# EthanD11/RS-VIO

Measured on AMD Instinct MI355X. Metric: stereo frames/sec (tracker+BA) on 752×480 EuRoC stream; BA ms/iter at window=10, higher is better.
Workload: dtype f32 (tracker) / f64 (BA)

## Files before the change

### rs-vio_amd/csrc/ba.hip

```cpp
#include <rccl/rccl.h>

#include <algorithm>
#include <chrono>
#include <cmath>
#include <cstdlib>
#include <cstring>
#include <string>
#include <sys/resource.h>
#include <numeric>
#include <stdexcept>
#include <vector>

#include "common.hpp"

#include "ba_envelope.hpp"
#include "obs_pass.hpp"
#include "se3.hpp"
#include "wave.hpp"

#pragma clang fp contract(fast)

namespace rsvio {

namespace {
// ... 1742 lines not shown
        __builtin_amdgcn_fence(__ATOMIC_ACQUIRE, "");
    }
    __syncthreads();
    const double* mine = p2p_slot(P.peer[me], par, 0);
    double sums[kE];
#pragma unroll
    for (int i = 0; i < kE; ++i) sums[i] = 0.0;
    if (nr <= 2)
        p2p_group_sums_own<kE, 2>(mine, nr, me, ne, tid, T, own, sums);
    else if (nr <= 4)
        p2p_group_sums_own<kE, 4>(mine, nr, me, ne, tid, T, own, sums);
    else
        p2p_group_sums_own<kE, 8>(mine, nr, me, ne, tid, T, own, sums);
#pragma unroll
    for (int i = 0; i < kE; ++i) {
        const int e = tid + T * i;
        if (e >= ne) break;
        const double a = sums[i];
        const int d = dst[i];
        if (d >= 0)
            M[d & (kMfMapLambda - 1)] = a;
        else if (d <= -2)
            gsh[-2 - d] = a;
    }
    if (tid == 0) {
        double cv[kP2PMax], fv[kP2PMax];
#pragma unroll
        for (int r = 0; r < kP2PMax; ++r) {
            const bool peer = r < nr && r != me;
            cv[r] = peer ? __hip_atomic_load(mine + (size_t)r * kP2PMsg + ne, __ATOMIC_RELAXED, __HIP_MEMORY_SCOPE_SYSTEM)
                         : osc[0];
            fv[r] = peer ? __hip_atomic_load(mine + (size_t)r * kP2PMsg + ne + 1, __ATOMIC_RELAXED,
                                             __HIP_MEMORY_SCOPE_SYSTEM)
                         : osc[1];
        }
        double c = 0.0, f = 0.0;
#pragma unroll
        for (int r = 0; r < kP2PMax; ++r)
            if (r < nr) {
                c += cv[r];
                f += fv[r];
            }
        Wk.sys[ne] = c;
        *fail = f != 0.0;
        *xgen = gen;
    }
    if (tid < nr && P.xnw)
        P.xnw[tid] = tid == me ? G.n_wave
                               : (int)__hip_atomic_load(mine + (size_t)tid * kP2PMsg + ne + 2, __ATOMIC_RELAXED,
                                                        __HIP_MEMORY_SCOPE_SYSTEM);
    return false;
}

template <int H, int J, int PW, bool KD = false>
__device__ __forceinline__ void mf_pivot(double (&a)[kMfPanel], double (&uq)[kMfPanel], double lp, double inv,
                                         double* Lf, double* Up, int lane, bool& bad, double* Dv = nullptr) {
    constexpr int K = kMfPanel * H + J;
    const double u = a[J];
    if constexpr (KD)
        if (lane == 0) Dv[K] = inv;
    double inv_next = 1.0;
    double uk1 = 0.0;
    if constexpr (J + 1 < PW) {
        uk1 = rl64(u, K + 1);
        const double piv = fma(-(uk1 * uk1), inv, rl64(a[J + 1], K + 1));
        bad |= !(piv > 0.0) || !isfinite(piv);
#ifndef RSVIO_K5_RCP_LATE
        double y0 = __builtin_amdgcn_rcp(piv);
        __asm__ volatile("" : "+v"(y0));
        const double e = fma(-piv, y0, 1.0);
        inv_next = fma(y0, fma(e, e, e), y0);
#else
        inv_next = rcp_f64(piv);
#endif
    }
    const double l = u * inv;
    if constexpr (J + 1 < PW) a[J + 1] = fma(-l, uk1, a[J + 1]);
    __builtin_amdgcn_sched_barrier(0);
    if constexpr (J > 0)
#pragma unroll
        for (int jj = J + 2; jj < PW; ++jj) a[jj] = fma(-lp, uq[jj], a[jj]);
    if constexpr (J + 2 < PW) a[J + 2] = fma(-l, rl64(u, K + 2), a[J + 2]);
    Lf[K * kMfLd + lane] = l;
    Up[J * kMfLd + lane] = u;
#ifndef RSVIO_K5_LDSQ
#pragma unroll
    for (int jj = J + 3; jj < PW; ++jj) uq[jj] = rl64(u, kMfPanel * H + jj);
#else
#pragma unroll
    for (int jj = J + 3; jj < PW; ++jj) uq[jj] = Up[J * kMfLd + kMfPanel * H + jj];
#endif
    if constexpr (J + 1 < PW) mf_pivot<H, J + 1, PW, KD>(a, uq, l, inv_next, Lf, Up, lane, bad, Dv);
}

template <int NF, int H, bool KD = false>
__device__ __forceinline__ void mf_factor(const double* M, double* Lf, double* Uh, int lane, bool& bad,
                                          double* Dv = nullptr) {
    constexpr int NP = MfDims<NF>::NP;
    constexpr int C0 = kMfPanel * H;
    constexpr int PW = (NP - C0) < kMfPanel ? (NP - C0) : kMfPanel;
    double a[kMfPanel], uq[kMfPanel];
#pragma unroll
    for (int jj = 0; jj < kMfPanel; ++jj) {
        a[jj] = jj < PW ? M[(C0 + jj) * kMfLd + lane] : 0.0;
        uq[jj] = 0.0;
    }
    const double piv = rl64(a[0], C0);
    bad |= !(piv > 0.0) || !isfinite(piv);
    mf_pivot<H, 0, PW, KD>(a, uq, 0.0, rcp_f64(piv), Lf, Uh, lane, bad, Dv);
}

template <int NF, int H>
__device__ __forceinline__ void mf_update(double* M, const double* Lf, const double* Uh, int lane, int wid, int nw,
                                          int J0, int J1) {
    constexpr int NT = MfDims<NF>::NT;
    constexpr int C0 = kMfPanel * H;
    const int i16 = lane & 15, k4 = lane >> 4;
    int ntile = 0;
    for (int J = J0; J < J1; ++J) ntile += NT - J;
    for (int t = wid; t < ntile; t += nw) {
        int TJ = J0, rem = t;
        while (rem >= NT - TJ) {
            rem -= NT - TJ;
            ++TJ;
        }
        const int TI = TJ + rem;
        double av[2], bv[2];
#pragma unroll
        for (int m = 0; m < 2; ++m) {
            const int kk = 4 * m + k4;
            av[m] = -Uh[kk * kMfLd + 16 * TI + i16];
            bv[m] = Lf[(C0 + kk) * kMfLd + 16 * TJ + i16];
        }
        mf_dbl4 c;
#pragma unroll
        for (int r = 0; r < 4; ++r) c[r] = M[(16 * TJ + i16) * kMfLd + 16 * TI + k4 + 4 * r];
        c = __builtin_amdgcn_mfma_f64_16x16x4f64(av[0], bv[0], c, 0, 0, 0);
        c = __builtin_amdgcn_mfma_f64_16x16x4f64(av[1], bv[1], c, 0, 0, 0);
#pragma unroll
        for (int r = 0; r < 4; ++r) M[(16 * TJ + i16) * kMfLd + 16 * TI + k4 + 4 * r] = c[r];
    }
}

template <int NF, int H, bool KD = false>
__device__ __forceinline__ void mf_panel(double* M, double* Lf, double* Up, int tid, bool& bad, double* Dv = nullptr) {
    constexpr int NT = MfDims<NF>::NT, NH = MfDims<NF>::NH;
    constexpr int C0 = kMfPanel * H;
    const int lane = tid & 63, wave = tid >> 6;
    if constexpr (H == 0) STAMP(9); else if constexpr (H == 2) STAMP(15); else if constexpr (H == 4) STAMP(30);
    if constexpr (H + 1 == NH) STAMP(7);
    if constexpr (H + 1 < NH) {
        constexpr int T0 = (C0 + kMfPanel) / 16;
        double* Uh = Up + (H & 1) * kMfPanel * kMfLd;
        if (wave == 0) {
            mf_update<NF, H>(M, Lf, Uh, lane, 0, 1, T0, T0 + 1);
            __builtin_amdgcn_fence(__ATOMIC_SEQ_CST, "wavefront");
            __builtin_amdgcn_wave_barrier();
            mf_factor<NF, H + 1, KD>(M, Lf, Up + ((H + 1) & 1) * kMfPanel * kMfLd, lane, bad, Dv);
        } else {
            mf_update<NF, H>(M, Lf, Uh, lane, wave - 1, kK5Threads / 64 - 1, T0 + 1, NT);
        }
        __syncthreads();
        if constexpr (H == 0) STAMP(13); else if constexpr (H == 2) STAMP(19); else if constexpr (H == 4) STAMP(31);
        mf_panel<NF, H + 1, KD>(M, Lf, Up, tid, bad, Dv);
    }
}

#ifdef RSVIO_STAMPS
#define WSTAMP(w, k)                                                                           \
    do {                                                                                       \
        if (threadIdx.x == 64 * (w) && blockIdx.x < 4096) {                                    \
            __builtin_amdgcn_s_waitcnt(0);                                                     \
            g_dbg[blockIdx.x * 32 + (k)] = (unsigned long long)clock64();                      \
        }                                                                                      \
    } while (0)
#else
#define WSTAMP(w, k) \
    do {             \
    } while (0)
#endif

template <int NF>
struct BkDims {
    static constexpr int NP = 6 * NF;
    static constexpr int RPL = NP + 1 <= 64 ? 1 : 2;
    static constexpr int NT = (NP + 1 + 15) / 16;
    static constexpr int NPP = 16 * NT;
    static constexpr int NTC = (NP + 15) / 16;
    static constexpr int LD = NF <= 10 ? kMfLd : kBkLd;
};

template <int NF, int K, int NWU>
__device__ __forceinline__ void bk_update(double* M, const double* Uk, int lane, int wid, int env) {
    using D = BkDims<NF>;
    constexpr int c0 = 6 * K, cmin = c0 + 12;
    if constexpr (cmin < D::NP) {
        constexpr int TJ0 = cmin / 16;
        constexpr int ntile_dense = (D::NTC - TJ0) * D::NT - (D::NTC - 1 + TJ0) * (D::NTC - TJ0) / 2;
        constexpr int Q = (ntile_dense + NWU - 1) / NWU;
        constexpr int TIb = D::NP / 16;
        const int rlast = min(6 * (env + 1), D::NP) - 1;
        const int TIe = rlast / 16;
        const int TJe = env >= K + 2 ? min(TIe, D::NTC - 1) : TJ0 - 1;
        const int extra = TIb > TIe ? 1 : 0;
        int ntile = 0;
        for (int TJ = TJ0; TJ <= TJe; ++TJ) ntile += TIe - TJ + 1 + extra;
        const int i16 = lane & 15, k4 = lane >> 4;
        double av[Q][2], bv[Q][2];
        mf_dbl4 c[Q];
        int base[Q];
        bool live[Q];
#pragma unroll
        for (int q = 0; q < Q; ++q) {
            const int t = wid + NWU * q;
            int TJ = TJ0, rem = t < ntile ? t : 0;
            while (rem >= TIe - TJ + 1 + extra) {
                rem -= TIe - TJ + 1 + extra;
                ++TJ;
            }
            const int TI = rem <= TIe - TJ ? TJ + rem : TIb;
            const int col = 16 * TJ + i16;
            live[q] = t < ntile && col >= cmin && col < D::NP;
            base[q] = col * D::LD + 16 * TI + k4;
#pragma unroll
            for (int m = 0; m < 2; ++m) {
                const int kk = 4 * m + k4;
                av[q][m] = kk < 6 ? -Uk[kk * D::LD + 16 * TI + i16] : 0.0;
                bv[q][m] = (kk < 6 && live[q]) ? M[(c0 + kk) * D::LD + col] : 0.0;
            }
#pragma unroll
            for (int r = 0; r < 4; ++r) c[q][r] = live[q] ? M[base[q] + 4 * r] : 0.0;
        }
#pragma unroll
        for (int q = 0; q < Q; ++q)
            if (wid + NWU * q < ntile) c[q] = __builtin_amdgcn_mfma_f64_16x16x4f64(av[q][0], bv[q][0], c[q], 0, 0, 0);
#pragma unroll
        for (int q = 0; q < Q; ++q)
            if (wid + NWU * q < ntile) c[q] = __builtin_amdgcn_mfma_f64_16x16x4f64(av[q][1], bv[q][1], c[q], 0, 0, 0);
#pragma unroll
        for (int q = 0; q < Q; ++q)
            if (live[q])
#pragma unroll
                for (int r = 0; r < 4; ++r) M[base[q] + 4 * r] = c[q][r];
    }
}

template <int NF, int K, int NW, bool KD = false>
__device__ __forceinline__ void bk_steps(double* M, double* U, double* Dsc, double* Lsc,
                                         double (&a)[BkDims<NF>::RPL][6], int tid, bool& bad,
                                         const unsigned char* env, double* Dv = nullptr) {
    using D = BkDims<NF>;
    constexpr int RPL = D::RPL, LD = D::LD, c0 = 6 * K;
    const int lane = tid & 63, wave = tid >> 6;
    double u[RPL][6];
    if constexpr (K < 9) WSTAMP(0, 8 + K);
    WSTAMP(0, 32 + K);
    WSTAMP(1, 64 + K);
    WSTAMP(7, 160 + K);
    if (wave == 0) {
        double Dg[6][6], Lg[6][6], inv[6];
#ifdef RSVIO_BK_DIAG_LDS
#pragma unroll
        for (int h = 0; h < RPL; ++h) {
            const int i = lane + 64 * h - c0;
            if (i >= 0 && i < 6)
#pragma unroll
                for (int j = 0; j < 6; ++j) Dsc[6 * i + j] = a[h][j];
        }
        __builtin_amdgcn_fence(__ATOMIC_SEQ_CST, "wavefront");
        __builtin_amdgcn_wave_barrier();
#pragma unroll
        for (int i = 0; i < 6; ++i)
#pragma unroll
            for (int j = 0; j <= i; ++j) Dg[i][j] = Dsc[6 * i + j];
#else
#pragma unroll
        for (int i = 0; i < 6; ++i)
#pragma unroll
            for (int j = 0; j <= i; ++j) Dg[i][j] = rl64(a[(c0 + i) >> 6][j], (c0 + i) & 63);
#endif
#pragma unroll
        for (int j = 0; j < 6; ++j) {
            const double piv = Dg[j][j];
            bad |= !(piv > 0.0) || !isfinite(piv);
            inv[j] = rcp_f64(piv);
#pragma unroll
            for (int i = j + 1; i < 6; ++i) Lg[i][j] = Dg[i][j] * inv[j];
#pragma unroll
            for (int i = j + 1; i < 6; ++i)
#pragma unroll
                for (int i2 = j + 1; i2 <= i; ++i2) Dg[i][i2] = fma(-Lg[i][j], Dg[i2][j], Dg[i][i2]);
        }
        if constexpr (KD)
            if (lane == 0)
#pragma unroll
                for (int j = 0; j < 6; ++j) Dv[c0 + j] = inv[j];
#pragma unroll
        for (int h = 0; h < RPL; ++h) {
            const int r = lane + 64 * h, i = r - c0;
            double t[6], l[6];
#pragma unroll
            for (int j = 0; j < 6; ++j) t[j] = a[h][j];
#pragma unroll
            for (int j = 0; j < 6; ++j) {
                u[h][j] = t[j];
                l[j] = t[j] * inv[j];
#pragma unroll
                for (int j2 = j + 1; j2 < 6; ++j2) t[j2] = fma(-l[j], Dg[j2][j], t[j2]);
            }
            const bool below = i >= 6 && r <= D::NP;
            if (i >= 0 && r <= D::NP)
// ... 3352 lines not shown
```

### rs-vio_amd/csrc/pyramid.hip

```cpp
#include "pyramid.hpp"

namespace rsvio {

namespace {

constexpr int TW = 64;
constexpr int TH = 8;
constexpr int STRIP_COLS = 320;
constexpr size_t LDS_CAP = 64 << 10;

__device__ __forceinline__ float triangle_kernel(float x) {
    float ax = fabsf(x);
    return ax < 1.0f ? 1.0f - ax : 0.0f;
}

__global__ void make_taps_kernel(TapTable tab, int n_entries) {
    int e = blockIdx.x * blockDim.x + threadIdx.x;
    if (e >= n_entries) return;
    int in_len = tab.ent_in_len[e];
    int out_len = tab.ent_out_len[e];
    int o = tab.ent_out_idx[e];
    float ratio = (float)in_len / (float)out_len;
    float sratio = ratio < 1.0f ? 1.0f : ratio;
    float support = 1.0f * sratio;
    float inputc = ((float)o + 0.5f) * ratio;
    long long left = (long long)floorf(inputc - support);
    if (left < 0) left = 0;
    if (left > (long long)in_len - 1) left = in_len - 1;
    long long right = (long long)ceilf(inputc + support);
    if (right < left + 1) right = left + 1;
    if (right > (long long)in_len) right = in_len;
    inputc = inputc - 0.5f;
    int cnt = (int)(right - left);
    float* w = tab.weights + (size_t)e * tab.max_taps;
    float sum = 0.0f;
    for (int k = 0; k < cnt; ++k) {
        float wv = triangle_kernel(((float)(left + k) - inputc) / sratio);
        w[k] = wv;
        sum += wv;
    }
    for (int k = 0; k < cnt; ++k) w[k] = w[k] / sum;
    tab.left[e] = (int)left;
    tab.count[e] = cnt;
}

__global__ __launch_bounds__(256) void pyramid_kernel(PyrLaunch L, PyrIO io) {
    extern __shared__ uint32_t smem[];
    const int img = blockIdx.y;
    {
        const int fb = (int)blockIdx.x - (L.copy_blocks + L.tile_start[L.levels]);
        if (fb >= 0) {
            if (img == 0 && fb < io.fast_cells) {
                const uint8_t* s0 = io.psrc ? io.psrc : io.src[0];
                fast_cell(s0, io.fg, fb, nullptr, nullptr, 0, io.fast_pt, io.fast_aff,
                          reinterpret_cast<uint8_t*>(smem));
            }
            return;
        }
    }
    const uint8_t* __restrict__ src = io.psrc ? io.psrc + (size_t)img * L.w * L.h : io.src[img];
    uint8_t* __restrict__ dst_base = io.psrc ? io.pdst + (size_t)img * L.pyr_bytes : io.dst[img];
    int b = blockIdx.x;
    const bool aligned = ((reinterpret_cast<uintptr_t>(src) | reinterpret_cast<uintptr_t>(dst_base)) & 15) == 0;
    if (b < L.copy_blocks) {
        const size_t tot = (size_t)L.w * L.h;
        if (!aligned) {
            for (size_t i = (size_t)b * blockDim.x + threadIdx.x; i < tot; i += (size_t)L.copy_blocks * blockDim.x)
                dst_base[i] = src[i];
            return;
        }
        const size_t n16 = tot / 16;
        const uint4* s4 = reinterpret_cast<const uint4*>(src);
        uint4* d4 = reinterpret_cast<uint4*>(dst_base);
        for (size_t i = (size_t)b * blockDim.x + threadIdx.x; i < n16; i += (size_t)L.copy_blocks * blockDim.x)
            d4[i] = s4[i];
        size_t tail0 = n16 * 16;
        if (b == 0)
            for (size_t i = tail0 + threadIdx.x; i < tot; i += blockDim.x) dst_base[i] = src[i];
        return;
    }
    b -= L.copy_blocks;
    int lev = 1;
    while (lev < L.levels - 1 && b >= L.tile_start[lev + 1]) ++lev;
    b -= L.tile_start[lev];
    const int nw = (int)level_w(L.w, lev), nh = (int)level_h(L.h, lev);
    const int tw = L.tile_w[lev], th = L.tile_h[lev];
    const int tiles_x = (nw + tw - 1) / tw;
    const int tx = b % tiles_x, ty = b / tiles_x;
    const int ox0 = tx * tw, ox1 = min(ox0 + tw, nw);
    const int oy0 = ty * th, oy1 = min(oy0 + th, nh);
    const int rows = oy1 - oy0, cols_out = ox1 - ox0;
    const int hx = L.hx_ent[lev], vy = L.vy_ent[lev];
    const TapTable& T = L.tab;
    const int xl = T.left[hx + ox0];
    const int xr = T.left[hx + ox1 - 1] + T.count[hx + ox1 - 1];
    const int yl = T.left[vy + oy0];
    const int yr = T.left[vy + oy1 - 1] + T.count[vy + oy1 - 1];
    const int ncols = xr - xl, nrows = yr - yl;
    const int xa = xl & ~3, xoff = xl - xa;
    const int pd = (xr - xa + 3) >> 2;
    const bool direct = (L.direct >> lev) & 1;
    uint8_t* strip = reinterpret_cast<uint8_t*>(smem);
    if (!direct) {
        if (aligned && (L.w & 3) == 0) {
            const uint32_t* s32 = reinterpret_cast<const uint32_t*>(src);
            const int wd = (int)(L.w >> 2);
            for (int idx = threadIdx.x; idx < nrows * pd; idx += blockDim.x) {
                const int r = idx / pd, d = idx - r * pd;
                smem[idx] = s32[(size_t)(yl + r) * wd + (xa >> 2) + d];
            }
        } else {
            for (int idx = threadIdx.x; idx < nrows * pd * 4; idx += blockDim.x) {
                const int r = idx / (pd * 4), c = idx - r * pd * 4;
                strip[idx] = (xa + c < (int)L.w) ? src[(size_t)(yl + r) * L.w + xa + c] : 0;
            }
        }
    }
    float* tmp = reinterpret_cast<float*>(smem + (direct ? 0 : nrows * pd));
    __syncthreads();
    for (int idx = threadIdx.x; idx < rows * ncols; idx += blockDim.x) {
        const int r = idx / ncols, c = idx - r * ncols;
        const int e = vy + oy0 + r;
        const int vl = T.left[e], vc = T.count[e];
        const float* __restrict__ vw = T.weights + (size_t)e * T.max_taps;
        float acc = 0.0f;
        if (!direct) {
            const uint8_t* col = strip + (vl - yl) * pd * 4 + xoff + c;
            for (int k = 0; k < vc; ++k) acc += (float)col[k * pd * 4] * vw[k];
        } else {
            const uint8_t* __restrict__ col = src + (size_t)vl * L.w + xl + c;
            for (int k = 0; k < vc; k += 8) {
                float px[8];
#pragma unroll
                for (int u = 0; u < 8; ++u) px[u] = (k + u < vc) ? (float)col[(size_t)(k + u) * L.w] : 0.0f;
#pragma unroll
                for (int u = 0; u < 8; ++u)
                    if (k + u < vc) acc += px[u] * vw[k + u];
            }
        }
        tmp[r * ncols + c] = acc;
    }
    __syncthreads();
    uint8_t* __restrict__ dst = dst_base + level_offset(L.w, L.h, lev);
    for (int idx = threadIdx.x; idx < rows * cols_out; idx += blockDim.x) {
        const int r = idx / cols_out, c = idx - r * cols_out;
        const int e = hx + ox0 + c;
        const int hl = T.left[e] - xl, hc = T.count[e];
        const float* __restrict__ hw = T.weights + (size_t)e * T.max_taps;
        const float* __restrict__ row = tmp + r * ncols + hl;
        float acc = 0.0f;
        for (int k = 0; k < hc; ++k) acc += row[k] * hw[k];
        float cl = acc < 0.0f ? 0.0f : (acc > 255.0f ? 255.0f : acc);
        dst[(size_t)(oy0 + r) * nw + ox0 + c] = (uint8_t)roundf(cl);
    }
}

}

void PyramidPlan::init(int w_, int h_, int levels_) {
    w = w_;
    h = h_;
    levels = levels_;
    if (levels < 1 || levels > kMaxLevels) throw std::invalid_argument("levels must be in [1, 8]");
    if (w < 16 || h < 16) throw std::invalid_argument("image too small");
    std::vector<int> in_len, out_len, out_idx;
    float max_ratio = 1.0f;
    memset(&launch, 0, sizeof(launch));
    for (int i = 1; i < levels; ++i) {
        int nw = (int)level_w(w, i), nh = (int)level_h(h, i);
        if (nw < 1 || nh < 1) throw std::invalid_argument("too many levels for image size");
        launch.hx_ent[i] = (int)in_len.size();
        for (int o = 0; o < nw; ++o) { in_len.push_back(w); out_len.push_back(nw); out_idx.push_back(o); }
        launch.vy_ent[i] = (int)in_len.size();
        for (int o = 0; o < nh; ++o) { in_len.push_back(h); out_len.push_back(nh); out_idx.push_back(o); }
        float rx = (float)w / nw, ry = (float)h / nh;
        max_ratio = std::max(max_ratio, std::max(rx, ry));
        launch.tile_h[i] = std::max(1, std::min(TH, (int)(16.0f / ry)));
        launch.tile_w[i] = std::max(1, std::min(TW, (int)std::floor((STRIP_COLS - 2.0f * rx - 4.0f) / rx)));
    }
    n_entries = (int)in_len.size();
    max_taps = (int)std::ceil(2.0f * max_ratio) + 4;
    int tiles = 0;
    for (int i = 1; i < levels; ++i) {
        launch.tile_start[i] = tiles;
        int nw = (int)level_w(w, i), nh = (int)level_h(h, i);
        tiles += ((nw + launch.tile_w[i] - 1) / launch.tile_w[i]) * ((nh + launch.tile_h[i] - 1) / launch.tile_h[i]);
    }
    launch.tile_start[levels] = tiles;
    launch.copy_blocks = std::max(1, (int)(((size_t)w * h / 16 + 255) / 256 / 4));
    total_blocks = launch.copy_blocks + tiles;
    launch.w = (uint32_t)w;
    launch.h = (uint32_t)h;
    launch.levels = levels;
    launch.pyr_bytes = level_offset(w, h, levels);
    if (n_entries > 0) {
        i_in.alloc(n_entries); i_out.alloc(n_entries); i_idx.alloc(n_entries);
        d_left.alloc(n_entries); d_count.alloc(n_entries);
        d_w.alloc((size_t)n_entries * max_taps);
        RSVIO_HIP(hipMemcpy(i_in.p, in_len.data(), sizeof(int) * n_entries, hipMemcpyHostToDevice));
        RSVIO_HIP(hipMemcpy(i_out.p, out_len.data(), sizeof(int) * n_entries, hipMemcpyHostToDevice));
        RSVIO_HIP(hipMemcpy(i_idx.p, out_idx.data(), sizeof(int) * n_entries, hipMemcpyHostToDevice));
        TapTable t;
        t.left = d_left.p; t.count = d_count.p; t.weights = d_w.p; t.max_taps = max_taps;
        t.ent_in_len = i_in.p; t.ent_out_len = i_out.p; t.ent_out_idx = i_idx.p;
        hipLaunchKernelGGL(make_taps_kernel, dim3((n_entries + 255) / 256), dim3(256), 0, 0, t, n_entries);
        RSVIO_HIP(hipGetLastError());
        RSVIO_HIP(hipDeviceSynchronize());
        launch.tab = t;
        std::vector<int> left(n_entries), count(n_entries);
        RSVIO_HIP(hipMemcpy(left.data(), d_left.p, sizeof(int) * n_entries, hipMemcpyDeviceToHost));
        RSVIO_HIP(hipMemcpy(count.data(), d_count.p, sizeof(int) * n_entries, hipMemcpyDeviceToHost));
        for (int i = 1; i < levels; ++i) {
            const int nw = (int)level_w(w, i), nh = (int)level_h(h, i);
            const int tw = launch.tile_w[i], th = launch.tile_h[i];
            size_t strip = 0, vert = 0;
            for (int ox0 = 0; ox0 < nw; ox0 += tw) {
                const int ox1 = std::min(ox0 + tw, nw);
                const int xl = left[launch.hx_ent[i] + ox0];
                const int xr = left[launch.hx_ent[i] + ox1 - 1] + count[launch.hx_ent[i] + ox1 - 1];
                const size_t pd = (size_t)(xr - (xl & ~3) + 3) / 4;
                for (int oy0 = 0; oy0 < nh; oy0 += th) {
                    const int oy1 = std::min(oy0 + th, nh);
                    const int yl = left[launch.vy_ent[i] + oy0];
                    const int yr = left[launch.vy_ent[i] + oy1 - 1] + count[launch.vy_ent[i] + oy1 - 1];
                    strip = std::max(strip, 4 * pd * (size_t)(yr - yl));
                    vert = std::max(vert, 4 * (size_t)(oy1 - oy0) * (size_t)(xr - xl));
                }
            }
            if (vert > LDS_CAP) throw std::invalid_argument("image too wide for the pyramid tile");
            if (strip + vert > LDS_CAP) launch.direct |= 1u << i;
            lds_bytes = std::max(lds_bytes, ((launch.direct >> i) & 1) ? vert : strip + vert);
        }
    }
}

void PyramidPlan::enqueue(const PyrIO& io, int n_img, hipStream_t s) const {
    if (n_img <= 0) return;
    if (n_img > (io.psrc ? 65535 : kMaxPyrIO)) throw std::invalid_argument("too many images per pyramid launch");
    const size_t lds = io.fast_cells > 0 ? std::max(lds_bytes, (size_t)io.fg.g * io.fg.g) : lds_bytes;
    hipLaunchKernelGGL(pyramid_kernel, dim3(total_blocks + std::max(io.fast_cells, 0), n_img), dim3(256), lds, s,
                       launch, io);
    RSVIO_HIP(hipGetLastError());
}

void PyramidPlan::enqueue(const uint8_t* d_imgs, int n_img, uint8_t* d_pyrs, hipStream_t s) const {
    for (int i0 = 0; i0 < n_img; i0 += 65535) {
        PyrIO io{};
        io.psrc = d_imgs + (size_t)i0 * w * h;
        io.pdst = d_pyrs + (size_t)i0 * pyr_bytes();
        enqueue(io, std::min(65535, n_img - i0), s);
    }
}

}
```

### rs-vio_amd/csrc/pyramid.hpp

```cpp
#pragma once
#include <algorithm>
#include <cmath>
#include <cstring>
#include <stdexcept>
#include <vector>

#include "common.hpp"
#include "fast.hpp"

namespace rsvio {

constexpr int kMaxLevels = 8;

struct TapTable {
    int* left = nullptr;
    int* count = nullptr;
    float* weights = nullptr;
    int max_taps = 0;
    const int* ent_in_len = nullptr;
    const int* ent_out_len = nullptr;
    const int* ent_out_idx = nullptr;
};

struct PyrLaunch {
    uint32_t w, h;
    int levels;
    size_t pyr_bytes;
    int copy_blocks;
    int tile_start[kMaxLevels + 1];
    int tile_w[kMaxLevels];
    int tile_h[kMaxLevels];
    uint32_t direct;
    int hx_ent[kMaxLevels];
    int vy_ent[kMaxLevels];
    TapTable tab;
};

constexpr int kMaxPyrIO = 8;
struct PyrIO {
    const uint8_t* src[kMaxPyrIO];
    uint8_t* dst[kMaxPyrIO];
    const uint8_t* psrc;
    uint8_t* pdst;
    int fast_cells;
    GridGeom fg;
    int4* fast_pt;
    float* fast_aff;
};

struct PyramidPlan {
    int w = 0, h = 0, levels = 0;
    int n_entries = 0, max_taps = 0, total_blocks = 0;
    size_t lds_bytes = 0;
    PyrLaunch launch;
    DevBuf<int> i_in, i_out, i_idx, d_left, d_count;
    DevBuf<float> d_w;
    void init(int w, int h, int levels);
    size_t pyr_bytes() const { return level_offset(w, h, levels); }
    void enqueue(const uint8_t* d_imgs, int n_img, uint8_t* d_pyrs, hipStream_t s) const;
    void enqueue(const PyrIO& io, int n_img, hipStream_t s) const;
};

}
```

### rs-vio_amd/rsvio/__init__.py

```python
from ._lib import RsvioError, load, require_device
from .tracker import (StereoPatchTracker, build_image_pyramid, detect_key_points,
                      pyramid_bytes, pyramid_levels, track_points)

__all__ = ["RsvioError", "load", "require_device", "StereoPatchTracker", "build_image_pyramid",
           "detect_key_points", "pyramid_bytes", "pyramid_levels", "track_points"]
```

### rs-vio_amd/rsvio/tracker.py

```python
from __future__ import annotations

import ctypes as C

import numpy as np

from . import _lib
from ._lib import check, ptr


def pyramid_bytes(w: int, h: int, levels: int) -> int:
    return int(_lib.load().rsvio_pyramid_bytes(w, h, levels))


def pyramid_levels(pyr: np.ndarray, w: int, h: int, levels: int) -> list[np.ndarray]:
    out, off = [], 0
    for i in range(levels):
        lw, lh = w // (1 << i), h // (1 << i)
        out.append(pyr[off:off + lw * lh].reshape(lh, lw))
        off += lw * lh
    return out


def build_image_pyramid(img: np.ndarray, levels: int) -> np.ndarray:
    img = np.ascontiguousarray(img, np.uint8)
    h, w = img.shape
    out = np.empty(pyramid_bytes(w, h, levels), np.uint8)
    check(_lib.load().rsvio_build_pyramid(ptr(img), w, h, levels, ptr(out)))
    return out


def track_points(pyr0: np.ndarray, pyr1: np.ndarray, w: int, h: int, levels: int, aff: np.ndarray,
                 max_iterations: int = 20, thresh: float = 0.01):
    aff = np.ascontiguousarray(aff, np.float32).reshape(-1, 6)
    n = aff.shape[0]
    out = np.empty_like(aff)
    valid = np.zeros(n, np.uint8)
    check(_lib.load().rsvio_track_points(ptr(pyr0), ptr(pyr1), w, h, levels, ptr(aff), n, max_iterations,
                                         C.c_float(thresh), ptr(out), ptr(valid)))
    return out, valid.astype(bool)


def detect_key_points(img: np.ndarray, grid_size: int, existing_xy: np.ndarray | None = None, cap: int = 4096):
    img = np.ascontiguousarray(img, np.uint8)
    h, w = img.shape
    ex = np.zeros((0, 2), np.float32) if existing_xy is None else np.ascontiguousarray(existing_xy, np.float32)
    out = np.zeros((cap, 2), np.uint32)
    score = np.zeros(cap, np.float32)
    n = C.c_int32(0)
    check(_lib.load().rsvio_detect_keypoints(ptr(img), w, h, grid_size, ptr(ex) if len(ex) else None, len(ex),
                                             ptr(out), ptr(score), cap, C.byref(n)))
    return out[:n.value].copy(), score[:n.value].copy()


FEATURE_DTYPE = np.dtype([("id", np.uint64), ("x", np.float32), ("y", np.float32), ("r", np.float32, 4)])


class StereoPatchTracker:

    def __init__(self, width: int, height: int, levels: int = 6, grid_size: int = 50,
                 optical_flow_max_iterations: int = 20, optical_flow_convergence_threshold: float = 0.01,
                 device: int = 0, max_features: int = 4096):
        lib = _lib.load()
        p = _lib.TrackerParams(width, height, levels, grid_size, optical_flow_max_iterations,
                               float(optical_flow_convergence_threshold), device, max_features)
        h = C.c_void_p()
        check(lib.rsvio_tracker_create(C.byref(p), C.byref(h)))
        self._h = h
        self.width, self.height, self.levels = width, height, levels
        self.cap = max_features
        self._out_l = np.zeros(max_features, FEATURE_DTYPE)
        self._out_r = np.zeros(max_features, FEATURE_DTYPE)
        self._n = (0, 0)

    def close(self):
        if getattr(self, "_h", None):
            _lib.load().rsvio_tracker_destroy(self._h)
            self._h = None

    def __del__(self):
        try:
            self.close()
        except Exception:
            pass

    def process_frame(self, left: np.ndarray, right: np.ndarray):
        left = np.ascontiguousarray(left, np.uint8)
        right = np.ascontiguousarray(right, np.uint8)
        if left.shape != (self.height, self.width) or right.shape != left.shape:
            raise ValueError(f"expected {self.height}x{self.width} images")
        nl, nr = C.c_size_t(0), C.c_size_t(0)
        rc = _lib.load().rsvio_tracker_process_frame(self._h, ptr(left), ptr(right), self.width,
                                                     ptr(self._out_l), self.cap, C.byref(nl),
                                                     ptr(self._out_r), self.cap, C.byref(nr))
        self._n = (nl.value, nr.value)
        check(rc)
        return self._out_l[:nl.value].copy(), self._out_r[:nr.value].copy()

    def process_frame_device(self, d_left: int, d_right: int):
        nl, nr = C.c_size_t(0), C.c_size_t(0)
        rc = _lib.load().rsvio_tracker_process_frame_device(self._h, d_left, d_right, ptr(self._out_l), self.cap,
                                                            C.byref(nl), ptr(self._out_r), self.cap, C.byref(nr))
        self._n = (nl.value, nr.value)
        check(rc)
        return nl.value, nr.value

    def submit(self, left: np.ndarray, right: np.ndarray):
        left = np.ascontiguousarray(left, np.uint8)
        right = np.ascontiguousarray(right, np.uint8)
        if left.shape != (self.height, self.width) or right.shape != left.shape:
            raise ValueError(f"expected {self.height}x{self.width} images")
        check(_lib.load().rsvio_tracker_submit(self._h, ptr(left), ptr(right), self.width))
        self._borrowed = (left, right)

    def submit_device(self, d_left: int, d_right: int):
        check(_lib.load().rsvio_tracker_submit_device(self._h, d_left, d_right))

    def collect_device(self):
        nl, nr = C.c_size_t(0), C.c_size_t(0)
        rc = _lib.load().rsvio_tracker_collect(self._h, ptr(self._out_l), self.cap, C.byref(nl), ptr(self._out_r),
                                               self.cap, C.byref(nr))
        self._n = (nl.value, nr.value)
        self._borrowed = None
        check(rc)
        return nl.value, nr.value

    def collect(self):
        nl, nr = self.collect_device()
        return self._out_l[:nl].copy(), self._out_r[:nr].copy()

    def get_track_points(self):
        l, r = self._out_l[:self._n[0]], self._out_r[:self._n[1]]
        return [{int(f["id"]): (float(f["x"]), float(f["y"])) for f in l},
                {int(f["id"]): (float(f["x"]), float(f["y"])) for f in r}]

    def set_cameras(self, left, right):
        if left is None:
            check(_lib.load().rsvio_tracker_set_cameras(self._h, None, None))
            self._cams = False
            return
        self._cl, self._cr = left.struct(), right.struct()
        check(_lib.load().rsvio_tracker_set_cameras(self._h, C.byref(self._cl), C.byref(self._cr)))
        self._cams = True

    def undistorted(self):
        ul = np.zeros((self._n[0], 2), np.float32)
        ur = np.zeros((self._n[1], 2), np.float32)
        check(_lib.load().rsvio_tracker_undistorted(self._h, ptr(ul), self._n[0], ptr(ur), self._n[1]))
        return ul, ur

    def remove_id(self, ids):
        ids = np.ascontiguousarray(ids, np.uint64)
        check(_lib.load().rsvio_tracker_remove_ids(self._h, ptr(ids), len(ids)))
        n = []
        for out, k in ((self._out_l, self._n[0]), (self._out_r, self._n[1])):
            keep = out[:k][~np.isin(out[:k]["id"], ids)]
            out[:len(keep)] = keep
            n.append(len(keep))
        self._n = tuple(n)
```

Baseline: 5071.

## Rework pyramid kernel to wave-strided tiles with LDS tap weights and recomputed spans

```diff
diff --git a/rs-vio_amd/csrc/ba.hip b/rs-vio_amd/csrc/ba.hip
--- a/rs-vio_amd/csrc/ba.hip
+++ b/rs-vio_amd/csrc/ba.hip
@@ -1918,11 +1918,19 @@
     if constexpr (H + 1 < NH) {
         constexpr int T0 = (C0 + kMfPanel) / 16;
         double* Uh = Up + (H & 1) * kMfPanel * kMfLd;
+#ifndef RSVIO_K5_LA_WAVE0
+        mf_update<NF, H>(M, Lf, Uh, lane, wave, kK5Threads / 64, T0, T0 + 1);
+        __syncthreads();
+#endif
         if (wave == 0) {
+#ifdef RSVIO_K5_LA_WAVE0
             mf_update<NF, H>(M, Lf, Uh, lane, 0, 1, T0, T0 + 1);
             __builtin_amdgcn_fence(__ATOMIC_SEQ_CST, "wavefront");
             __builtin_amdgcn_wave_barrier();
+#endif
+            if constexpr (H < 5) STAMP(20 + H);
             mf_factor<NF, H + 1, KD>(M, Lf, Up + ((H + 1) & 1) * kMfPanel * kMfLd, lane, bad, Dv);
+            if constexpr (H == 0) STAMP(25); else if constexpr (H == 2) STAMP(8); else if constexpr (H == 4) STAMP(10);
         } else {
             mf_update<NF, H>(M, Lf, Uh, lane, wave - 1, kK5Threads / 64 - 1, T0 + 1, NT);
         }
diff --git a/rs-vio_amd/csrc/pyramid.hip b/rs-vio_amd/csrc/pyramid.hip
--- a/rs-vio_amd/csrc/pyramid.hip
+++ b/rs-vio_amd/csrc/pyramid.hip
@@ -14,12 +14,8 @@
     return ax < 1.0f ? 1.0f - ax : 0.0f;
 }
 
-__global__ void make_taps_kernel(TapTable tab, int n_entries) {
-    int e = blockIdx.x * blockDim.x + threadIdx.x;
-    if (e >= n_entries) return;
-    int in_len = tab.ent_in_len[e];
-    int out_len = tab.ent_out_len[e];
-    int o = tab.ent_out_idx[e];
+__device__ __forceinline__ void tap_span(int in_len, int out_len, int o, int& left_out, int& cnt_out, float& inputc_out,
+                                         float& sratio_out) {
     float ratio = (float)in_len / (float)out_len;
     float sratio = ratio < 1.0f ? 1.0f : ratio;
     float support = 1.0f * sratio;
@@ -30,8 +26,25 @@
     long long right = (long long)ceilf(inputc + support);
     if (right < left + 1) right = left + 1;
     if (right > (long long)in_len) right = in_len;
-    inputc = inputc - 0.5f;
-    int cnt = (int)(right - left);
+    inputc_out = inputc - 0.5f;
+    sratio_out = sratio;
+    left_out = (int)left;
+    cnt_out = (int)(right - left);
+}
+__device__ __forceinline__ void tap_span(int in_len, int out_len, int o, int& left, int& cnt) {
+    float ic, sr;
+    tap_span(in_len, out_len, o, left, cnt, ic, sr);
+}
+
+__global__ void make_taps_kernel(TapTable tab, int n_entries) {
+    int e = blockIdx.x * blockDim.x + threadIdx.x;
+    if (e >= n_entries) return;
+    int in_len = tab.ent_in_len[e];
+    int out_len = tab.ent_out_len[e];
+    int o = tab.ent_out_idx[e];
+    int left, cnt;
+    float inputc, sratio;
+    tap_span(in_len, out_len, o, left, cnt, inputc, sratio);
     float* w = tab.weights + (size_t)e * tab.max_taps;
     float sum = 0.0f;
     for (int k = 0; k < cnt; ++k) {
@@ -40,15 +53,17 @@
         sum += wv;
     }
     for (int k = 0; k < cnt; ++k) w[k] = w[k] / sum;
-    tab.left[e] = (int)left;
+    tab.left[e] = left;
     tab.count[e] = cnt;
 }
 
+__host__ __device__ inline int align4(int n) { return (n + 3) & ~3; }
+
 __global__ __launch_bounds__(256) void pyramid_kernel(PyrLaunch L, PyrIO io) {
-    extern __shared__ uint32_t smem[];
+    extern __shared__ __attribute__((aligned(16))) uint32_t smem[];
     const int img = blockIdx.y;
     {
-        const int fb = (int)blockIdx.x - (L.copy_blocks + L.tile_start[L.levels]);
+        const int fb = (int)blockIdx.x - (L.copy_blocks + L.n_tiles);
         if (fb >= 0) {
             if (img == 0 && fb < io.fast_cells) {
                 const uint8_t* s0 = io.psrc ? io.psrc : io.src[0];
@@ -81,77 +96,105 @@
     }
     b -= L.copy_blocks;
     int lev = 1;
-    while (lev < L.levels - 1 && b >= L.tile_start[lev + 1]) ++lev;
-    b -= L.tile_start[lev];
-    const int nw = (int)level_w(L.w, lev), nh = (int)level_h(L.h, lev);
-    const int tw = L.tile_w[lev], th = L.tile_h[lev];
-    const int tiles_x = (nw + tw - 1) / tw;
-    const int tx = b % tiles_x, ty = b / tiles_x;
+#pragma unroll
+    for (int l = 2; l < kMaxLevels; ++l)
+        if (l < L.levels && b >= L.lv[l].tile_start) lev = l;
+    const PyrLevel& V = L.lv[lev];
+    b -= V.tile_start;
+    const int lane = threadIdx.x & 63, wave = threadIdx.x >> 6;
+    const int w = (int)L.w, h = (int)L.h;
+    const int nw = V.nw, nh = V.nh, tw = V.tile_w, th = V.tile_h;
+    const int ty = b / V.tiles_x, tx = b - ty * V.tiles_x;
     const int ox0 = tx * tw, ox1 = min(ox0 + tw, nw);
     const int oy0 = ty * th, oy1 = min(oy0 + th, nh);
     const int rows = oy1 - oy0, cols_out = ox1 - ox0;
-    const int hx = L.hx_ent[lev], vy = L.vy_ent[lev];
-    const TapTable& T = L.tab;
-    const int xl = T.left[hx + ox0];
-    const int xr = T.left[hx + ox1 - 1] + T.count[hx + ox1 - 1];
-    const int yl = T.left[vy + oy0];
-    const int yr = T.left[vy + oy1 - 1] + T.count[vy + oy1 - 1];
-    const int ncols = xr - xl, nrows = yr - yl;
-    const int xa = xl & ~3, xoff = xl - xa;
-    const int pd = (xr - xa + 3) >> 2;
+    int xl, yl, xe, ye, ce;
+    tap_span(w, nw, ox0, xl, ce);
+    tap_span(w, nw, ox1 - 1, xe, ce);
+    const int xr = xe + ce;
+    tap_span(h, nh, oy0, yl, ce);
+    tap_span(h, nh, oy1 - 1, ye, ce);
+    const int yr = ye + ce;
+    const int nrows = yr - yl;
+    const int xa = xl & ~3;
+    const int pd = (xr - xa + 3) >> 2, pd4 = pd * 4;
     const bool direct = (L.direct >> lev) & 1;
-    uint8_t* strip = reinterpret_cast<uint8_t*>(smem);
+    const int ktv = V.kt_v, kth = V.kt_h;
+    float* vW = reinterpret_cast<float*>(smem);
+    float* hW = vW + align4(th * ktv);
+    uint32_t* strip32 = smem + align4(th * ktv) + align4(kth * tw);
+    float* tmp = reinterpret_cast<float*>(strip32 + (direct ? 0 : align4(nrows * pd)));
+    {
+        const float* __restrict__ Wt = L.tab.weights;
+        const int mt = L.tab.max_taps;
+        for (int r = wave; r < rows; r += 4)
+            for (int k = lane; k < ktv; k += 64) vW[r * ktv + k] = Wt[(size_t)(V.vy_ent + oy0 + r) * mt + k];
+        if (lane < cols_out)
+            for (int k = wave; k < kth; k += 4) hW[k * tw + lane] = Wt[(size_t)(V.hx_ent + ox0 + lane) * mt + k];
+    }
     if (!direct) {
-        if (aligned && (L.w & 3) == 0) {
-            const uint32_t* s32 = reinterpret_cast<const uint32_t*>(src);
-            const int wd = (int)(L.w >> 2);
-            for (int idx = threadIdx.x; idx < nrows * pd; idx += blockDim.x) {
-                const int r = idx / pd, d = idx - r * pd;
-                smem[idx] = s32[(size_t)(yl + r) * wd + (xa >> 2) + d];
+        if (aligned && (w & 3) == 0) {
+            const uint32_t* __restrict__ s32 = reinterpret_cast<const uint32_t*>(src);
+            const int wd = w >> 2;
+            for (int r = wave; r < nrows; r += 4)
+                for (int d = lane; d < pd; d += 64) strip32[r * pd + d] = s32[(size_t)(yl + r) * wd + (xa >> 2) + d];
+        } else {
+            uint8_t* strip = reinterpret_cast<uint8_t*>(strip32);
+            for (int r = wave; r < nrows; r += 4)
+                for (int c = lane; c < pd4; c += 64)
+                    strip[r * pd4 + c] = (xa + c < w) ? src[(size_t)(yl + r) * w + xa + c] : 0;
+        }
+    }
+    __syncthreads();
+    for (int r = wave; r < rows; r += 4) {
+        int vl, vc;
+        tap_span(h, nh, oy0 + r, vl, vc);
+        const float* vw = vW + r * ktv;
+        if (!direct) {
+            const uint32_t* col = strip32 + (vl - yl) * pd;
+            for (int d = lane; d < pd; d += 64) {
+                float a0 = 0.0f, a1 = 0.0f, a2 = 0.0f, a3 = 0.0f;
+                for (int k = 0; k < vc; ++k) {
+                    const uint32_t p = col[k * pd + d];
+                    const float wk = vw[k];
+                    a0 += (float)(p & 255u) * wk;
+                    a1 += (float)((p >> 8) & 255u) * wk;
+                    a2 += (float)((p >> 16) & 255u) * wk;
+                    a3 += (float)(p >> 24) * wk;
+                }
+                *reinterpret_cast<float4*>(tmp + r * pd4 + 4 * d) = make_float4(a0, a1, a2, a3);
             }
         } else {
-            for (int idx = threadIdx.x; idx < nrows * pd * 4; idx += blockDim.x) {
-                const int r = idx / (pd * 4), c = idx - r * pd * 4;
-                strip[idx] = (xa + c < (int)L.w) ? src[(size_t)(yl + r) * L.w + xa + c] : 0;
+            for (int c = lane; c < pd4; c += 64) {
+                float acc = 0.0f;
+                if (xa + c < w) {
+                    const uint8_t* __restrict__ col = src + (size_t)vl * w + xa + c;
+                    for (int k = 0; k < vc; k += 8) {
+                        float px[8];
+#pragma unroll
+                        for (int u = 0; u < 8; ++u) px[u] = (k + u < vc) ? (float)col[(size_t)(k + u) * w] : 0.0f;
+#pragma unroll
+                        for (int u = 0; u < 8; ++u)
+                            if (k + u < vc) acc += px[u] * vw[k + u];
+                    }
+                }
+                tmp[r * pd4 + c] = acc;
             }
         }
     }
-    float* tmp = reinterpret_cast<float*>(smem + (direct ? 0 : nrows * pd));
     __syncthreads();
-    for (int idx = threadIdx.x; idx < rows * ncols; idx += blockDim.x) {
-        const int r = idx / ncols, c = idx - r * ncols;
-        const int e = vy + oy0 + r;
-        const int vl = T.left[e], vc = T.count[e];
-        const float* __restrict__ vw = T.weights + (size_t)e * T.max_taps;
-        float acc = 0.0f;
-        if (!direct) {
-            const uint8_t* col = strip + (vl - yl) * pd * 4 + xoff + c;
-            for (int k = 0; k < vc; ++k) acc += (float)col[k * pd * 4] * vw[k];
-        } else {
-            const uint8_t* __restrict__ col = src + (size_t)vl * L.w + xl + c;
-            for (int k = 0; k < vc; k += 8) {
-                float px[8];
-#pragma unroll
-                for (int u = 0; u < 8; ++u) px[u] = (k + u < vc) ? (float)col[(size_t)(k + u) * L.w] : 0.0f;
-#pragma unroll
-                for (int u = 0; u < 8; ++u)
-                    if (k + u < vc) acc += px[u] * vw[k + u];
-            }
-        }
-        tmp[r * ncols + c] = acc;
-    }
-    __syncthreads();
-    uint8_t* __restrict__ dst = dst_base + level_offset(L.w, L.h, lev);
-    for (int idx = threadIdx.x; idx < rows * cols_out; idx += blockDim.x) {
-        const int r = idx / cols_out, c = idx - r * cols_out;
-        const int e = hx + ox0 + c;
-        const int hl = T.left[e] - xl, hc = T.count[e];
-        const float* __restrict__ hw = T.weights + (size_t)e * T.max_taps;
-        const float* __restrict__ row = tmp + r * ncols + hl;
-        float acc = 0.0f;
-        for (int k = 0; k < hc; ++k) acc += row[k] * hw[k];
-        float cl = acc < 0.0f ? 0.0f : (acc > 255.0f ? 255.0f : acc);
-        dst[(size_t)(oy0 + r) * nw + ox0 + c] = (uint8_t)roundf(cl);
+    if (lane < cols_out) {
+        int hl, hc;
+        tap_span(w, nw, ox0 + lane, hl, hc);
+        uint8_t* __restrict__ dst = dst_base + V.off;
+        const float* hw = hW + lane;
+        for (int r = wave; r < rows; r += 4) {
+            const float* row = tmp + r * pd4 + (hl - xa);
+            float acc = 0.0f;
+            for (int k = 0; k < hc; ++k) acc += row[k] * hw[k * tw];
+            float cl = acc < 0.0f ? 0.0f : (acc > 255.0f ? 255.0f : acc);
+            dst[(size_t)(oy0 + r) * nw + ox0 + lane] = (uint8_t)roundf(cl);
+        }
     }
 }
 
@@ -167,26 +210,31 @@
     float max_ratio = 1.0f;
     memset(&launch, 0, sizeof(launch));
     for (int i = 1; i < levels; ++i) {
+        PyrLevel& V = launch.lv[i];
         int nw = (int)level_w(w, i), nh = (int)level_h(h, i);
         if (nw < 1 || nh < 1) throw std::invalid_argument("too many levels for image size");
-        launch.hx_ent[i] = (int)in_len.size();
+        V.nw = nw;
+        V.nh = nh;
+        V.off = level_offset(w, h, i);
+        V.hx_ent = (int)in_len.size();
         for (int o = 0; o < nw; ++o) { in_len.push_back(w); out_len.push_back(nw); out_idx.push_back(o); }
-        launch.vy_ent[i] = (int)in_len.size();
+        V.vy_ent = (int)in_len.size();
         for (int o = 0; o < nh; ++o) { in_len.push_back(h); out_len.push_back(nh); out_idx.push_back(o); }
         float rx = (float)w / nw, ry = (float)h / nh;
         max_ratio = std::max(max_ratio, std::max(rx, ry));
-        launch.tile_h[i] = std::max(1, std::min(TH, (int)(16.0f / ry)));
-        launch.tile_w[i] = std::max(1, std::min(TW, (int)std::floor((STRIP_COLS - 2.0f * rx - 4.0f) / rx)));
+        V.tile_h = std::max(1, std::min(TH, (int)(16.0f / ry)));
+        V.tile_w = std::max(1, std::min(TW, (int)std::floor((STRIP_COLS - 2.0f * rx - 4.0f) / rx)));
     }
     n_entries = (int)in_len.size();
     max_taps = (int)std::ceil(2.0f * max_ratio) + 4;
     int tiles = 0;
     for (int i = 1; i < levels; ++i) {
-        launch.tile_start[i] = tiles;
-        int nw = (int)level_w(w, i), nh = (int)level_h(h, i);
-        tiles += ((nw + launch.tile_w[i] - 1) / launch.tile_w[i]) * ((nh + launch.tile_h[i] - 1) / launch.tile_h[i]);
-    }
-    launch.tile_start[levels] = tiles;
+        PyrLevel& V = launch.lv[i];
+        V.tile_start = tiles;
+        V.tiles_x = (V.nw + V.tile_w - 1) / V.tile_w;
+        tiles += V.tiles_x * ((V.nh + V.tile_h - 1) / V.tile_h);
+    }
+    launch.n_tiles = tiles;
     launch.copy_blocks = std::max(1, (int)(((size_t)w * h / 16 + 255) / 256 / 4));
     total_blocks = launch.copy_blocks + tiles;
     launch.w = (uint32_t)w;
@@ -211,25 +259,29 @@
         RSVIO_HIP(hipMemcpy(left.data(), d_left.p, sizeof(int) * n_entries, hipMemcpyDeviceToHost));
         RSVIO_HIP(hipMemcpy(count.data(), d_count.p, sizeof(int) * n_entries, hipMemcpyDeviceToHost));
         for (int i = 1; i < levels; ++i) {
-            const int nw = (int)level_w(w, i), nh = (int)level_h(h, i);
-            const int tw = launch.tile_w[i], th = launch.tile_h[i];
+            PyrLevel& V = launch.lv[i];
+            const int nw = V.nw, nh = V.nh, tw = V.tile_w, th = V.tile_h;
+            for (int o = 0; o < nw; ++o) V.kt_h = std::max(V.kt_h, count[V.hx_ent + o]);
+            for (int o = 0; o < nh; ++o) V.kt_v = std::max(V.kt_v, count[V.vy_ent + o]);
+            if (V.kt_h > max_taps || V.kt_v > max_taps) throw std::logic_error("pyramid: tap count past the table's row");
+            const size_t taps = 4 * ((size_t)align4(th * V.kt_v) + (size_t)align4(V.kt_h * tw));
             size_t strip = 0, vert = 0;
             for (int ox0 = 0; ox0 < nw; ox0 += tw) {
                 const int ox1 = std::min(ox0 + tw, nw);
-                const int xl = left[launch.hx_ent[i] + ox0];
-                const int xr = left[launch.hx_ent[i] + ox1 - 1] + count[launch.hx_ent[i] + ox1 - 1];
+                const int xl = left[V.hx_ent + ox0];
+                const int xr = left[V.hx_ent + ox1 - 1] + count[V.hx_ent + ox1 - 1];
                 const size_t pd = (size_t)(xr - (xl & ~3) + 3) / 4;
                 for (int oy0 = 0; oy0 < nh; oy0 += th) {
                     const int oy1 = std::min(oy0 + th, nh);
-                    const int yl = left[launch.vy_ent[i] + oy0];
-                    const int yr = left[launch.vy_ent[i] + oy1 - 1] + count[launch.vy_ent[i] + oy1 - 1];
-                    strip = std::max(strip, 4 * pd * (size_t)(yr - yl));
-                    vert = std::max(vert, 4 * (size_t)(oy1 - oy0) * (size_t)(xr - xl));
+                    const int yl = left[V.vy_ent + oy0];
+                    const int yr = left[V.vy_ent + oy1 - 1] + count[V.vy_ent + oy1 - 1];
+                    strip = std::max(strip, 4 * (size_t)align4((int)pd * (yr - yl)));
+                    vert = std::max(vert, 4 * (size_t)(oy1 - oy0) * 4 * pd);
                 }
             }
-            if (vert > LDS_CAP) throw std::invalid_argument("image too wide for the pyramid tile");
-            if (strip + vert > LDS_CAP) launch.direct |= 1u << i;
-            lds_bytes = std::max(lds_bytes, ((launch.direct >> i) & 1) ? vert : strip + vert);
+            if (taps + vert > LDS_CAP) throw std::invalid_argument("image too wide for the pyramid tile");
+            if (taps + strip + vert > LDS_CAP) launch.direct |= 1u << i;
+            lds_bytes = std::max(lds_bytes, taps + (((launch.direct >> i) & 1) ? vert : strip + vert));
         }
     }
 }
diff --git a/rs-vio_amd/csrc/pyramid.hpp b/rs-vio_amd/csrc/pyramid.hpp
--- a/rs-vio_amd/csrc/pyramid.hpp
+++ b/rs-vio_amd/csrc/pyramid.hpp
@@ -22,18 +22,25 @@
     const int* ent_out_idx = nullptr;
 };
 
+struct PyrLevel {
+    int tile_start;
+    int tiles_x;
+    int tile_w, tile_h;
+    int nw, nh;
+    int kt_h, kt_v;
+    int hx_ent, vy_ent;
+    size_t off;
+};
+
 struct PyrLaunch {
     uint32_t w, h;
     int levels;
+    int copy_blocks;
+    int n_tiles;
+    uint32_t direct;
     size_t pyr_bytes;
-    int copy_blocks;
-    int tile_start[kMaxLevels + 1];
-    int tile_w[kMaxLevels];
-    int tile_h[kMaxLevels];
-    uint32_t direct;
-    int hx_ent[kMaxLevels];
-    int vy_ent[kMaxLevels];
     TapTable tab;
+    PyrLevel lv[kMaxLevels];
 };
 
 constexpr int kMaxPyrIO = 8;
diff --git a/rs-vio_amd/rsvio/__init__.py b/rs-vio_amd/rsvio/__init__.py
--- a/rs-vio_amd/rsvio/__init__.py
+++ b/rs-vio_amd/rsvio/__init__.py
@@ -1,6 +1,6 @@
 from ._lib import RsvioError, load, require_device
-from .tracker import (StereoPatchTracker, build_image_pyramid, detect_key_points,
+from .tracker import (PyramidContext, StereoPatchTracker, build_image_pyramid, detect_key_points,
                       pyramid_bytes, pyramid_levels, track_points)
 
-__all__ = ["RsvioError", "load", "require_device", "StereoPatchTracker", "build_image_pyramid",
+__all__ = ["RsvioError", "load", "require_device", "PyramidContext", "StereoPatchTracker", "build_image_pyramid",
            "detect_key_points", "pyramid_bytes", "pyramid_levels", "track_points"]
diff --git a/rs-vio_amd/rsvio/tracker.py b/rs-vio_amd/rsvio/tracker.py
--- a/rs-vio_amd/rsvio/tracker.py
+++ b/rs-vio_amd/rsvio/tracker.py
@@ -27,6 +27,29 @@
     out = np.empty(pyramid_bytes(w, h, levels), np.uint8)
     check(_lib.load().rsvio_build_pyramid(ptr(img), w, h, levels, ptr(out)))
     return out
+
+
+class PyramidContext:
+
+    def __init__(self, w: int, h: int, levels: int, device: int = 0):
+        self.w, self.h, self.levels = w, h, levels
+        self._h = C.c_void_p()
+        check(_lib.load().rsvio_track_ctx_create(w, h, levels, device, C.byref(self._h)))
+
+    def build(self, d_imgs: int, n_img: int, d_pyrs: int, stream: int = 0) -> None:
+        check(_lib.load().rsvio_build_pyramids_d(self._h, C.c_void_p(d_imgs), n_img, C.c_void_p(d_pyrs),
+                                                 C.c_void_p(stream)))
+
+    def close(self):
+        if self._h:
+            _lib.load().rsvio_track_ctx_destroy(self._h)
+            self._h = C.c_void_p()
+
+    def __del__(self):
+        try:
+            self.close()
+        except Exception:
+            pass
 
 
 def track_points(pyr0: np.ndarray, pyr1: np.ndarray, w: int, h: int, levels: int, aff: np.ndarray,
```

New measurement: 5100, median of 4. No clear change (+0.6%).
